# snuspl/rnb

Hardware: AMD Instinct MI355X
Metric: videos/sec (whole node) + p50/p99 end-to-end latency, R(2+1)D-34 8-frame clips (higher is better)
Workload: dtype fp32

## Files before the change

### csrc/conv_h3.hip

```cpp
#include <type_traits>
#include <hip/hip_runtime.h>
#include <stdint.h>

#include "x6d_common.h"

#include "h3_common.h"

#ifdef H3_PHASE_TIMING
__device__ unsigned long long* h3_phase_buf;
#define H3_PHASE(k)                                                                   \
  do {                                                                                \
    if (threadIdx.x == 0 && (k) < 16) {                                               \
      h3_phase_buf[(size_t)blockIdx.x * 16 + (k)] = __builtin_amdgcn_s_memtime();     \
      if ((k) == 0) {                                                                 \
        unsigned hw, xcc;                                                             \
        asm volatile("s_getreg_b32 %0, hwreg(HW_REG_HW_ID)" : "=s"(hw));              \
        asm volatile("s_getreg_b32 %0, hwreg(HW_REG_XCC_ID)" : "=s"(xcc));            \
        h3_phase_buf[(size_t)blockIdx.x * 16 + 14] = ((unsigned long long)xcc << 32) | hw; \
      }                                                                               \
    }                                                                                 \
  } while (0)
#else
#define H3_PHASE(k) do {} while (0)
#endif
// ... 764 lines not shown
      rd_w(wh[0], wl[0], half * G, 0);
#pragma unroll
      for (int j = 0; j < G; ++j) {
        if (t0 + j >= 9) break;
        const bool more = j + 1 < G && t0 + j + 1 < 9;
#pragma unroll
        for (int tc = 0; tc < TC; ++tc) {
          const int cs = (j * TC + tc) & 1;
          if (tc + 1 < TC) rd_w(wh[cs ^ 1], wl[cs ^ 1], half * G + j, tc + 1);
          else if (more) rd_w(wh[cs ^ 1], wl[cs ^ 1], half * G + j + 1, 0);
          if (more && tc >= 1 && tc <= TP) rd_bf(bf[(j + 1) & 1][tc - 1], t0 + j + 1, tc - 1);
          const H3B (&b)[TP] = bf[j & 1];
#pragma unroll
          for (int tp = 0; tp < TP; ++tp) acc[tp][tc] = h3_mma(wl[cs], b[tp].h, acc[tp][tc]);
#pragma unroll
          for (int tp = 0; tp < TP; ++tp) acc[tp][tc] = h3_mma(wh[cs], b[tp].l, acc[tp][tc]);
#pragma unroll
          for (int tp = 0; tp < TP; ++tp) acc[tp][tc] = h3_mma(wh[cs], b[tp].h, acc[tp][tc]);
          __builtin_amdgcn_sched_barrier(0);
        }
      }
      x6d_wait_vm<0>();
      x6d_barrier();
      half ^= 1;
    }
    H3_PHASE(2 + 2 * c);
  }
  x6d_epilogue<TP, TC, NW, C_TILE, ST, STK>(p, st, acc, p0, m_end, p0 + P_TILE, c0, wave, 0,
                                            lane, lds, HALO_BYTES + 2 * G * W_BYTES,
                                            st.out_scale);
  H3_PHASE(15);
}

template <int NW, int TP, int TC, int HALO, int WB, int MINB, bool ST, bool AFF>
__global__ __launch_bounds__(64 * NW, MINB)
void conv_h3t_kernel(const ConvF32Params p, const X6DStats st) {
  constexpr int ROWS = NW * TP * 16, C_TILE = TC * 16;
  constexpr int HALO_BYTES = HALO * 128;
  constexpr int TAP_BYTES = C_TILE * 128;
  constexpr int W_BYTES = 3 * TAP_BYTES;
  constexpr int W_TOTAL = W_BYTES / 1024;
  constexpr int W_INSTR = (W_TOTAL + NW - 1) / NW;
  constexpr int NT = 64 * NW;
  constexpr int ITEMS = (HALO * 4 + NT - 1) / NT;
  static_assert(NT % 4 == 0 && TAP_BYTES % 1024 == 0, "staging / DMA split");
  static_assert(TP <= TC * 3 - 1, "next-tap fragments are read during the channel tiles");
  __shared__ __attribute__((aligned(16))) char lds[HALO_BYTES + WB * W_BYTES];
  char* const wbuf = lds + HALO_BYTES;

  const int lane = threadIdx.x & 63;
  const int wave = __builtin_amdgcn_readfirstlane(threadIdx.x >> 6);
  const int frow = lane & 15, fq = lane >> 4;
  const int T = p.T, HW = p.H * p.W, P = p.ngroups;
  const int nck = (p.Cin_p + 31) / 32;

  const int nwg = gridDim.x, bid = blockIdx.x;
  const int q8 = nwg >> 3, r8 = nwg & 7, xcd = bid & 7;
  const int wgid = (xcd < r8 ? xcd * (q8 + 1) : r8 * (q8 + 1) + (xcd - r8) * q8) + (bid >> 3);
  const int ctile = wgid % p.n_ctiles;
  const int rest = wgid / p.n_ctiles;
  const int ptile = rest % p.n_ptiles;
  const int n = rest / p.n_ptiles;
  const int c0 = ctile * C_TILE, hw0 = ptile * P;

  const x6d_u32x4 wr = x6d_rsrc(p.w, (uint32_t)(p.K_pad / 32) * (uint32_t)p.w_rows * 128u);
  auto issue_w = [&](int c, int buf) {
#pragma unroll
    for (int j = 0; j < W_INSTR; ++j) {
      const int instr = (W_TOTAL % NW == 0) ? wave + NW * j : min(wave + NW * j, W_TOTAL - 1);
      const int k = instr / (TAP_BYTES / 1024), part = instr % (TAP_BYTES / 1024);
      const uint32_t s = (uint32_t)(k * nck + c);
      x6d_dma16(wr, (s * (uint32_t)p.w_rows + (uint32_t)c0) * 128u +
                        (uint32_t)(part * 1024 + lane * 16),
                wbuf + buf * W_BYTES + instr * 1024);
    }
  };

  const __amdgpu_buffer_rsrc_t xr =
      __builtin_amdgcn_make_buffer_rsrc((void*)p.x, (short)0, p.x_bytes, 0x00020000);
  const int nent = (T + 2) * P;
  const int qd = threadIdx.x & 3;
  uint32_t src[ITEMS];
  int dst[ITEMS];
#pragma unroll
  for (int i = 0; i < ITEMS; ++i) {
    const int it = threadIdx.x + i * NT;
    const int e = it >> 2;
    const int fr = e / P - 1, px = e - (fr + 1) * P;
    const bool ok = it < 4 * nent && fr >= 0 && fr < T && hw0 + px < HW;
    src[i] = ok ? (uint32_t)((((n * T + fr) * HW + hw0 + px) * p.Cin_p + qd * 4) * 4) : X6D_INVALID;
    dst[i] = it < 4 * nent ? e * 128 : -1;
  }
  const float* ssv = nullptr;
  if constexpr (AFF) ssv = st.in_ss + (size_t)st.in_seg[n] * 2 * p.Cin_p + qd * 4;
  const float in_scale = st.in_scale;
  x6f32x4 raw0[ITEMS], raw1[ITEMS];
  auto load_chunk = [&](int c) {
    const bool hi_ok = c * 32 + 16 < p.Cin_p;
#pragma unroll
    for (int i = 0; i < ITEMS; ++i) {
      const uint32_t o = src[i] == X6D_INVALID ? X6D_INVALID : src[i] + (uint32_t)(c * 128);
      raw0[i] = __builtin_amdgcn_raw_buffer_load_b128(xr, o, 0, 0);
      raw1[i] = __builtin_amdgcn_raw_buffer_load_b128(xr, (o == X6D_INVALID || !hi_ok) ? X6D_INVALID
                                                                                  : o + 64u, 0, 0);
    }
  };
  auto store_chunk = [&](int c) {
    x6f32x4 sc0, sh0, sc1, sh1;
    if constexpr (AFF) {
      const bool hi_ok = c * 32 + 16 < p.Cin_p;
      const float* ss = ssv + c * 32;
      sc0 = *(const x6f32x4*)ss;
      sh0 = *(const x6f32x4*)(ss + p.Cin_p);
      sc1 = hi_ok ? *(const x6f32x4*)(ss + 16) : (x6f32x4){0.f, 0.f, 0.f, 0.f};
      sh1 = hi_ok ? *(const x6f32x4*)(ss + p.Cin_p + 16) : (x6f32x4){0.f, 0.f, 0.f, 0.f};
    }
#pragma unroll
    for (int i = 0; i < ITEMS; ++i) {
      if (dst[i] < 0) continue;
      const int e = dst[i] >> 7;
      x6f32x4 a0 = raw0[i], a1 = raw1[i];
      if constexpr (AFF) {
        const float m = src[i] == X6D_INVALID ? 0.f : in_scale;
#pragma unroll
        for (int j = 0; j < 4; ++j) {
          a0[j] = fmaxf(fmaf(a0[j], sc0[j], sh0[j]), 0.f) * m;
          a1[j] = fmaxf(fmaf(a1[j], sc1[j], sh1[j]), 0.f) * m;
        }
      } else {
        a0 *= in_scale;
        a1 *= in_scale;
      }
      uint32_t h[4], l[4];
      h3_split4(a0, h, l);
      h3_split4(a1, h + 2, l + 2);
      char* base = lds + dst[i];
      *(wu32x4*)(base + (x6r_swz(2 * qd, e) << 4)) = (wu32x4){h[0], h[1], h[2], h[3]};
      *(wu32x4*)(base + (x6r_swz(2 * qd + 1, e) << 4)) = (wu32x4){l[0], l[1], l[2], l[3]};
    }
  };

  int pe[TP];
#pragma unroll
  for (int tp = 0; tp < TP; ++tp) {
    const int r = (wave * TP + tp) * 16 + frow;
    const int fr = r / P;
    pe[tp] = fr * P + (r - fr * P);
  }

  x6f32x4 acc[TP][TC];
#pragma unroll
  for (int b = 0; b < TC; ++b) {
    const int c = c0 + b * 16 + 4 * fq;
    const float4 b4 = *(const float4*)(p.bias + c);
    const x6f32x4 bv = (x6f32x4){b4.x, b4.y, b4.z, b4.w} * st.acc_scale;
#pragma unroll
    for (int a = 0; a < TP; ++a) acc[a][b] = bv;
  }
  const int w_hh = x6_chunk(2 * fq, frow) << 4, w_ll = x6_chunk(2 * fq + 1, frow) << 4;
  auto rd_bf = [&](H3B& b, int k, int tp) {
    const int e = pe[tp] + k * P;
    const char* base = lds + e * 128;
    b.h = *(const wu32x4*)(base + (x6r_swz(2 * fq, e) << 4));
    b.l = *(const wu32x4*)(base + (x6r_swz(2 * fq + 1, e) << 4));
  };
  auto rd_w = [&](wu32x4& ah, wu32x4& al, int buf, int k, int tc) {
    const char* wrow = wbuf + buf * W_BYTES + k * TAP_BYTES + (tc * 16 + frow) * 128;
    ah = *(const wu32x4*)(wrow + w_hh);
    al = *(const wu32x4*)(wrow + w_ll);
  };

  int buf = 0;
  auto taps = [&]() {
    H3B bf[2][TP];
    wu32x4 wh[2], wl[2];
#pragma unroll
    for (int tp = 0; tp < TP; ++tp) rd_bf(bf[0][tp], 0, tp);
    rd_w(wh[0], wl[0], buf, 0, 0);
#pragma unroll
    for (int k = 0; k < 3; ++k) {
#pragma unroll
      for (int tc = 0; tc < TC; ++tc) {
        const int cs = (k * TC + tc) & 1;
        if (tc + 1 < TC) rd_w(wh[cs ^ 1], wl[cs ^ 1], buf, k, tc + 1);
        else if (k + 1 < 3) rd_w(wh[cs ^ 1], wl[cs ^ 1], buf, k + 1, 0);
        if (k + 1 < 3) {
#pragma unroll
          for (int tp = 0; tp < TP; ++tp)
            if (tp * TC / TP == tc && tp < TP) rd_bf(bf[(k + 1) & 1][tp], k + 1, tp);
        }
        const H3B (&b)[TP] = bf[k & 1];
#pragma unroll
        for (int tp = 0; tp < TP; ++tp) acc[tp][tc] = h3_mma(wl[cs], b[tp].h, acc[tp][tc]);
#pragma unroll
        for (int tp = 0; tp < TP; ++tp) acc[tp][tc] = h3_mma(wh[cs], b[tp].l, acc[tp][tc]);
#pragma unroll
        for (int tp = 0; tp < TP; ++tp) acc[tp][tc] = h3_mma(wh[cs], b[tp].h, acc[tp][tc]);
        __builtin_amdgcn_sched_barrier(0);
      }
    }
  };
  issue_w(0, 0);
  load_chunk(0);
  for (int c = 0; c < nck; ++c) {
    if (c > 0) x6d_barrier();
    if (WB == 1 && c > 0) issue_w(c, 0);
    store_chunk(c);
    x6d_wait_vm<0>();
    x6d_barrier();
    if (c + 1 < nck) {
      if (WB == 2) issue_w(c + 1, (c + 1) & 1);
      load_chunk(c + 1);
    }
    buf = WB == 2 ? (c & 1) : 0;
    taps();
  }

  const float out_scale = st.out_scale;
  const uint32_t y_bytes = (uint32_t)p.M * (uint32_t)p.y_stride * 4u;
  const __amdgpu_buffer_rsrc_t yr =
      __builtin_amdgcn_make_buffer_rsrc((void*)p.y, (short)0, y_bytes, 0x00020000);
  const bool has_res = p.res != nullptr;
  const __amdgpu_buffer_rsrc_t rr = __builtin_amdgcn_make_buffer_rsrc(
      (void*)(has_res ? p.res : p.y), (short)0,
      has_res ? (uint32_t)p.M * (uint32_t)p.res_stride * 4u : 0u, 0x00020000);
  int mrow[TP];
#pragma unroll
  for (int tp = 0; tp < TP; ++tp) {
    const int r = (wave * TP + tp) * 16 + frow;
    const int fr = r / P, px = r - fr * P;
    mrow[tp] = hw0 + px < HW ? (n * T + fr) * HW + hw0 + px : -1;
  }
  double* red = (double*)lds;
  bool bad = false;
  if constexpr (ST) {
    x6d_barrier();
    for (int i = threadIdx.x; i < C_TILE * 2; i += NT) red[i] = 0.0;
    __syncthreads();
  }
#pragma unroll
  for (int tc = 0; tc < TC; ++tc) {
    const int cl = tc * 16 + 4 * fq, c = c0 + cl;
    x6f32x4 rv[TP];
#pragma unroll
    for (int tp = 0; tp < TP; ++tp) {
      const bool ok = has_res && mrow[tp] >= 0 && c < p.Cout_p;
      rv[tp] = has_res ? __builtin_amdgcn_raw_buffer_load_b128(
                             rr, ok ? (uint32_t)(mrow[tp] * p.res_stride + c) * 4u : X6D_INVALID,
                             0, 0)
                       : (x6f32x4){0.f, 0.f, 0.f, 0.f};
    }
    float s1[4] = {0.f, 0.f, 0.f, 0.f}, s2[4] = {0.f, 0.f, 0.f, 0.f};
#pragma unroll
    for (int tp = 0; tp < TP; ++tp) {
      const bool ok = mrow[tp] >= 0 && c < p.Cout_p;
      x6f32x4 v = acc[tp][tc] * out_scale + rv[tp];
      if (st.oflag != nullptr && ok) bad |= x6d_nonfinite(v);
      if (p.relu) {
#pragma unroll
        for (int j = 0; j < 4; ++j) v[j] = fmaxf(v[j], 0.f);
      }
      __builtin_amdgcn_raw_buffer_store_b128(
          v, yr, ok ? (uint32_t)(mrow[tp] * p.y_stride + c) * 4u : X6D_INVALID, 0, 0);
      if (ST && ok) {
#pragma unroll
        for (int j = 0; j < 4; ++j) {
          s1[j] += v[j];
// ... 330 lines not shown
  f32_magic_div((uint32_t)p.Ho, &p.mHo, &p.sHo);
  f32_magic_div((uint32_t)p.To, &p.mTo, &p.sTo);
  f32_magic_div((uint32_t)p.H + 1u, &p.mG, &p.sG);
  p.ST = R;
  p.n_ctiles = (p.Cout_p + 143) / 144;
  if (p.n_ctiles * 144 > p.w_rows) return -8;
  const long long blocks = rnb_conv_h3r_blocks(variant, p.N, p.T, p.H, p.W, p.Cout_p);
  if (blocks > 0x7FFFFFFF) return -7;
  if (sums && (!clip_seg || stats_c < p.Cout_p)) return -12;
  X6DStats st;
  st.sums = sums;
  st.clip_seg = clip_seg;
  st.stats_c = stats_c;
  st.ksplit = 1;
  st.ws = nullptr;
  st.in_scale = in_scale;
  st.out_scale = out_scale;
  st.acc_scale = 1.f / out_scale;
  st.in_ss = in_ss;
  st.in_seg = in_seg;
  st.oflag = g_h3_range_flag;
  const int kid = (sums ? 1 : 0) + (in_ss ? 2 : 0);
  hipLaunchKernelGGL(stacked ? cfg.stacked[kid] : cfg.kernel[kid], dim3((unsigned)blocks),
                     dim3(64 * cfg.nw), 0, stream, p, st);
  return (int)hipGetLastError();
}

struct ConvH3TConfig {
  int rows, c_tile, halo, nw;
  void (*kernel)(const ConvF32Params, const X6DStats);
  void (*kernel_st)(const ConvF32Params, const X6DStats);
  void (*kernel_aff)(const ConvF32Params, const X6DStats);
  void (*kernel_aff_st)(const ConvF32Params, const X6DStats);
};
#define H3TCFG(NW, TP, TC, HALO, WB, MINB)                                         \
  {NW * TP * 16, TC * 16, HALO, NW,                                                  \
   conv_h3t_kernel<NW, TP, TC, HALO, WB, MINB, false, false>,                       \
   conv_h3t_kernel<NW, TP, TC, HALO, WB, MINB, true, false>,                        \
   conv_h3t_kernel<NW, TP, TC, HALO, WB, MINB, false, true>,                        \
   conv_h3t_kernel<NW, TP, TC, HALO, WB, MINB, true, true>}
static const ConvH3TConfig kH3TConfigs[] = {
    H3TCFG(8, 4, 4, 768, 2, 1), H3TCFG(8, 2, 4, 512, 2, 1), H3TCFG(8, 2, 8, 512, 2, 1),
    H3TCFG(4, 4, 4, 384, 1, 2),
};

int rnb_conv_h3t_num_variants() { return (int)(sizeof(kH3TConfigs) / sizeof(kH3TConfigs[0])); }

int rnb_conv_h3t_pixels(int variant, int T) {
  if (variant < 0 || variant >= rnb_conv_h3t_num_variants() || T < 2) return 0;
  const ConvH3TConfig& cfg = kH3TConfigs[variant];
  if (cfg.rows % T) return 0;
  const int P = cfg.rows / T;
  return (P % 16 == 0 && (T + 2) * P <= cfg.halo) ? P : 0;
}

int rnb_conv_h3t_launch(const ConvF32Params* pp, int variant, hipStream_t stream, double* sums,
                        const int* clip_seg, int stats_c, float in_scale, float out_scale,
                        const float* in_ss, const int* in_seg) {
  if (variant < 0 || variant >= rnb_conv_h3t_num_variants()) return -1;
  ConvF32Params p = *pp;
  const ConvH3TConfig& cfg = kH3TConfigs[variant];
  if (p.KT != 3 || p.KH != 1 || p.KW != 1 || p.PT != 1 || p.PH != 0 || p.PW != 0) return -2;
  if (p.ST != 1 || p.SH != 1 || p.SW != 1 || p.Cin_p % 16 != 0 || p.Cout_p % 4 != 0) return -2;
  const int nck = (p.Cin_p + 31) / 32;
  if (p.K_pad != 3 * 32 * nck) return -3;
  if (p.M <= 0) return 0;
  if (p.M != p.N * p.T * p.H * p.W) return -3;
  if (p.y_stride < p.Cout_p || p.y_stride % 4 != 0 || (p.res && (p.res_stride < p.Cout_p ||
                                                               p.res_stride % 4 != 0)))
    return -4;
  const long long xb = (long long)p.N * p.T * p.H * p.W * p.Cin_p * 4;
  if (xb > 0x7FFFFF00LL || (long long)p.M * p.y_stride * 4 > 0x7FFFFF00LL) return -5;
  if (p.res && (long long)p.M * p.res_stride * 4 > 0x7FFFFF00LL) return -6;
  const int P = rnb_conv_h3t_pixels(variant, p.T);
  if (P == 0) return -13;
  if ((long long)(p.K_pad / 32) * p.w_rows * 128 > 0x7FFFFF00LL) return -11;
  if (!(in_scale > 0.f) || !(out_scale > 0.f)) return -15;
  if (in_ss && !in_seg) return -16;
  p.x_bytes = (uint32_t)xb;
  p.ngroups = P;
  p.n_ptiles = (p.H * p.W + P - 1) / P;
  p.n_ctiles = (p.Cout_p + cfg.c_tile - 1) / cfg.c_tile;
  if (p.n_ctiles * cfg.c_tile > p.w_rows) return -8;
  const long long blocks = (long long)p.N * p.n_ptiles * p.n_ctiles;
  if (blocks > 0x7FFFFFFF) return -7;
  if (sums && (!clip_seg || stats_c < p.Cout_p)) return -12;
  X6DStats st;
  st.sums = sums;
  st.clip_seg = clip_seg;
  st.stats_c = stats_c;
  st.ksplit = 1;
  st.ws = nullptr;
  st.in_scale = in_scale;
  st.out_scale = out_scale;
  st.acc_scale = 1.f / out_scale;
  st.in_ss = in_ss;
  st.in_seg = in_seg;
  st.oflag = g_h3_range_flag;
  const bool aff = in_ss != nullptr;
  hipLaunchKernelGGL(aff ? (sums ? cfg.kernel_aff_st : cfg.kernel_aff)
                         : (sums ? cfg.kernel_st : cfg.kernel),
                     dim3((unsigned)blocks), dim3(64 * cfg.nw), 0, stream, p, st);
  return (int)hipGetLastError();
}

}
```

### rnb_amd/ops/conv_f32.py

```python
from __future__ import annotations

import math
import os
from typing import Dict, Optional, Tuple

import torch
import torch.nn.functional as F

from . import tuning
from .conv import ConvGeom, pad_to

F32_ALIGN = 4
F32_BK = 32
F32_ROW_SLACK = 256


_DEV_NAMES: Dict[int, str] = {}


def _device_name(device) -> str:
    if device is None or getattr(device, "type", "cpu") != "cuda":
        return "cpu"
    idx = device.index if device.index is not None else torch.cuda.current_device()
    if idx not in _DEV_NAMES:
# ... 390 lines not shown
            b[:self.geom.cout] = self.bias[:self.geom.cout].cpu()
            sw = h3_weight_scale_log2(w)
            self._h3d = (h3_direct_weights(w, sw).to(self.device), b.to(self.device),
                         float(2.0 ** H3_IN_LOG2), float(2.0 ** -(H3_IN_LOG2 + sw)))
        return self._h3d

    @property
    def h3t_k_pad(self) -> int:
        return 3 * 32 * ((self.geom.cin_p + 31) // 32)

    def h3t_buffers(self):
        if self.geom.cin_p % 32 == 0:
            return self.h3d_buffers()
        if self._h3t is None:
            rows, cin, kp = self.geom.cout_p + X6_ROW_SLACK, self.geom.cin_p, self.h3t_k_pad
            w = torch.zeros(rows, kp, dtype=torch.float32)
            tap = kp // 3
            src = self.wmat[:self.geom.cout, :self.k_total].cpu()
            for k in range(3):
                w[:self.geom.cout, k * tap:k * tap + cin] = src[:, k * cin:(k + 1) * cin]
            b = torch.zeros(rows, dtype=torch.float32)
            b[:self.geom.cout] = self.bias[:self.geom.cout].cpu()
            sw = h3_weight_scale_log2(w)
            self._h3t = (h3_direct_weights(w, sw).to(self.device), b.to(self.device),
                         float(2.0 ** H3_IN_LOG2), float(2.0 ** -(H3_IN_LOG2 + sw)))
        return self._h3t

    def h3t_ok(self, x_shape=None) -> bool:
        return (self.winot_ok and self.geom.cin_p % 16 == 0
                and (x_shape is None or x_shape[1] >= 2))

    def h3t_fits(self, variant: int, x_shape) -> bool:
        from .native import kernels
        return x_shape is None or kernels().conv_h3t_pixels(variant, x_shape[1]) > 0

    def h3p_ok(self, x_shape=None) -> bool:
        if not self.h3t_ok(x_shape) or os.environ.get("RNB_H3P", "1") == "0":
            return False
        from .native import kernels
        if x_shape is None:
            return kernels().conv_h3p_ok(8, 16, 16, self.geom.cin_p, self.geom.cout_p)
        _, T, H, W, _ = x_shape
        return kernels().conv_h3p_ok(T, H, W, self.geom.cin_p, self.geom.cout_p)

    def h3u_fits(self, variant: int, x_shape) -> bool:
        from .native import kernels
        return x_shape is None or kernels().conv_h3u_pixels(variant, x_shape[1]) > 0

    def wino_u(self, tc: int, m: int = 2, co0: int = 0, nco: Optional[int] = None,
               x6: bool = False) -> torch.Tensor:
        nco = self.geom.cout_p - co0 if nco is None else nco
        key = (m, tc, co0, nco, x6)
        u = self._wino_u.get(key)
        if u is None:
            fn = {2: winograd_weights, -4: winograd_t_weights}[m]
            w = self.w_ref[co0:co0 + nco].cpu()
            if w.shape[1] < self.geom.cin_p:
                w = torch.cat([w, w.new_zeros((w.shape[0], self.geom.cin_p - w.shape[1])
                                              + tuple(w.shape[2:]))], dim=1)
            u = self._wino_u[key] = fn(w, nco, tc, x6=x6).to(self.device)
        return u

    def h3w_u(self, tc: int) -> Tuple[torch.Tensor, int]:
        got = self._h3w.get(tc)
        if got is None:
            u, sw = h3w_weights(self.w_ref, self.geom.cin_p, self.geom.cout_p, tc)
            got = self._h3w[tc] = (u.to(self.device), sw)
# ... 643 lines not shown
```

### rnb_amd/ops/native.py

```python
from __future__ import annotations

import ctypes
import os
import struct
import threading
from typing import Optional

_HERE = os.path.dirname(os.path.abspath(__file__))
NATIVE_DIR = os.path.join(os.path.dirname(_HERE), "_native")

_lock = threading.Lock()
_libs = {}


class NativeUnavailable(RuntimeError):
    pass


def _lib_path(name: str) -> str:
    return os.path.join(NATIVE_DIR, name)


def _load(name: str, build_if_missing: bool = True) -> ctypes.CDLL:
    with _lock:
# ... 324 lines not shown
                                            ctypes.c_void_p, ctypes.c_void_p,
                                            ctypes.c_void_p, ctypes.c_int]
        lib.rnb_conv_x6r_launch.restype = ctypes.c_int
        lib.rnb_conv_x6_config_info.argtypes = [ctypes.c_int, ctypes.POINTER(ctypes.c_int),
                                                ctypes.POINTER(ctypes.c_int)]
        lib.rnb_conv_h3_launch.argtypes = [ctypes.POINTER(ConvParams), ctypes.c_int,
                                           ctypes.c_void_p, ctypes.c_void_p, ctypes.c_void_p,
                                           ctypes.c_int, ctypes.c_int, ctypes.c_void_p,
                                           ctypes.c_float, ctypes.c_float, ctypes.c_void_p,
                                           ctypes.c_void_p]
        lib.rnb_conv_h3_launch.restype = ctypes.c_int
        lib.rnb_conv_h3_affine_ok.argtypes = [ctypes.c_int, ctypes.c_int, ctypes.c_int]
        lib.rnb_conv_h3_affine_ok.restype = ctypes.c_int
        lib.rnb_conv_h3r_launch.argtypes = [ctypes.POINTER(ConvParams), ctypes.c_int,
                                            ctypes.c_void_p, ctypes.c_void_p, ctypes.c_void_p,
                                            ctypes.c_int, ctypes.c_float, ctypes.c_float,
                                            ctypes.c_void_p, ctypes.c_void_p]
        lib.rnb_conv_h3r_launch.restype = ctypes.c_int
        lib.rnb_conv_h3r_band_rows.argtypes = [ctypes.c_int] * 3
        lib.rnb_conv_h3r_band_rows.restype = ctypes.c_int
        lib.rnb_conv_h3r_pixels.argtypes = [ctypes.c_int]
        lib.rnb_conv_h3r_pixels.restype = ctypes.c_int
        lib.rnb_conv_h3r_blocks.argtypes = [ctypes.c_int] * 6
        lib.rnb_conv_h3r_blocks.restype = ctypes.c_longlong
        lib.rnb_conv_h3r_stacked.argtypes = [ctypes.c_int] * 6
        lib.rnb_conv_h3r_stacked.restype = ctypes.c_int
        lib.rnb_conv_h3r_stack_small.argtypes = [ctypes.c_int]
        lib.rnb_conv_h3r_stack_small.restype = None
        lib.rnb_conv_h3r_occupancy.argtypes = [ctypes.c_int] * 2
        lib.rnb_conv_h3r_occupancy.restype = ctypes.c_int
        lib.rnb_conv_h3t_launch.argtypes = lib.rnb_conv_h3r_launch.argtypes
        lib.rnb_conv_h3t_launch.restype = ctypes.c_int
        lib.rnb_conv_h3t_pixels.argtypes = [ctypes.c_int, ctypes.c_int]
        self.exp = None
        exp_path = os.path.join(NATIVE_DIR, "exp", "librnb_h3exp.so")
        if os.path.exists(exp_path) and os.environ.get("RNB_EXP_KERNELS", "1") != "0":
            try:
                self.exp = ctypes.CDLL(exp_path)
            except OSError:
                self.exp = None
        if self.exp is not None:
            ex = self.exp
            ex.rnb_conv_h3u_launch.argtypes = lib.rnb_conv_h3r_launch.argtypes
            ex.rnb_conv_h3u_launch.restype = ctypes.c_int
            ex.rnb_conv_h3u_pixels.argtypes = [ctypes.c_int, ctypes.c_int]
            ex.rnb_conv_h3u_pixels.restype = ctypes.c_int
            ex.rnb_conv_h3s_launch.argtypes = [ctypes.POINTER(ConvParams), ctypes.c_int,
                                               ctypes.c_void_p, ctypes.c_void_p,
                                               ctypes.c_void_p, ctypes.c_int, ctypes.c_float,
                                               ctypes.c_float]
            ex.rnb_conv_h3s_launch.restype = ctypes.c_int
            ex.rnb_conv_h3s_rows.argtypes = [ctypes.c_int, ctypes.c_int, ctypes.c_int]
            ex.rnb_conv_h3s_rows.restype = ctypes.c_int
        lib.rnb_conv_h3stem_launch.argtypes = [ctypes.POINTER(ConvParams), ctypes.c_int,
                                               ctypes.c_void_p, ctypes.c_void_p,
                                               ctypes.c_void_p, ctypes.c_int, ctypes.c_float,
                                               ctypes.c_float]
        lib.rnb_conv_h3stem_launch.restype = ctypes.c_int
        lib.rnb_conv_h3stem_rows.argtypes = [ctypes.c_int, ctypes.c_int, ctypes.c_int]
        lib.rnb_conv_h3stem_rows.restype = ctypes.c_int
        lib.rnb_conv_h3p_launch.argtypes = [ctypes.POINTER(ConvParams), ctypes.c_int,
                                            ctypes.c_void_p, ctypes.c_void_p, ctypes.c_void_p,
                                            ctypes.c_int, ctypes.c_float, ctypes.c_float,
                                            ctypes.c_void_p, ctypes.c_void_p]
        lib.rnb_conv_h3p_launch.restype = ctypes.c_int
        lib.rnb_conv_h3p_ok.argtypes = [ctypes.c_int] * 5
# ... 158 lines not shown

    def conv_h3p(self, params: ConvParams, blocks_per_cu: int, stream: int, in_scale: float,
                 out_scale: float, sums: int = 0, clip_seg: int = 0, stats_c: int = 0,
                 in_ss: int = 0, in_seg: int = 0) -> None:
        _check(self.lib.rnb_conv_h3p_launch(ctypes.byref(params), blocks_per_cu, stream,
                                            sums or None, clip_seg or None, stats_c, in_scale,
                                            out_scale, in_ss or None, in_seg or None),
               "conv_h3p (%d blocks per CU)" % blocks_per_cu)

    def conv_h3w(self, params: "WinoParams", variant: int, stream: int, in_scale: float,
                 out_scale: float, out_seg: int = 0) -> None:
        _check(self.lib.rnb_conv_h3w_launch(ctypes.byref(params), variant, stream, in_scale,
                                            out_scale, out_seg or None),
               "conv_h3w (variant %d)" % variant)

    def conv_h3w_tc(self, variant: int) -> int:
        return int(self.lib.rnb_conv_h3w_tc(variant))

    def conv_h3p_ok(self, T: int, H: int, W: int, Cin_p: int, Cout_p: int) -> bool:
        return bool(self.lib.rnb_conv_h3p_ok(T, H, W, Cin_p, Cout_p))

    def conv_h3stem_rows(self, variant: int, Ho: int, Wo: int) -> int:
        return int(self.lib.rnb_conv_h3stem_rows(variant, Ho, Wo))

    def conv_h3s_rows(self, variant: int, Ho: int, Wo: int) -> int:
        return int(self.exp.rnb_conv_h3s_rows(variant, Ho, Wo)) if self.exp else 0

    def conv_h3u_pixels(self, variant: int, T: int) -> int:
        return int(self.exp.rnb_conv_h3u_pixels(variant, T)) if self.exp else 0

    def conv_h3t_pixels(self, variant: int, T: int) -> int:
        return int(self.lib.rnb_conv_h3t_pixels(variant, T))

    def conv_h3_affine_ok(self, config_id: int, cin_p: int, rows_per_clip: int) -> bool:
        return bool(self.lib.rnb_conv_h3_affine_ok(config_id, cin_p, rows_per_clip))

    def conv_x6r(self, params: ConvParams, variant: int, stream: int, sums: int = 0,
                 clip_seg: int = 0, stats_c: int = 0) -> None:
        _check(self.lib.rnb_conv_x6r_launch(ctypes.byref(params), variant, stream,
                                            sums or None, clip_seg or None, stats_c),
               "conv_x6r (variant %d)" % variant)

    def wino_f32(self, params: "WinoParams", variant: int, stream: int) -> None:
        _check(self.lib.rnb_wino_f32_launch(ctypes.byref(params), variant, stream),
               "conv_wino_f32 (variant %d)" % variant)

    def winot_f32(self, params: "WinoParams", variant: int, stream: int) -> None:
        _check(self.lib.rnb_winot_f32_launch(ctypes.byref(params), variant, stream),
               "conv_winot_f32 (variant %d)" % variant)

    def wino_x6(self, params: "WinoParams", variant: int, stream: int) -> None:
        _check(self.lib.rnb_wino_x6_launch(ctypes.byref(params), variant, stream),
               "conv_wino_x6 (variant %d)" % variant)

    def winot_x6(self, params: "WinoParams", variant: int, stream: int) -> None:
        _check(self.lib.rnb_winot_x6_launch(ctypes.byref(params), variant, stream),
               "conv_winot_x6 (variant %d)" % variant)

    def preprocess_f32(self, in_ptr, out_ptr, npix, mean, std, stream):
        m = (ctypes.c_float * 3)(*mean)
        s = (ctypes.c_float * 3)(*std)
        _check(self.lib.rnb_preprocess_f32(in_ptr, out_ptr, npix, m, s, stream),
               "preprocess_f32")

    def head_f32(self, x_ptr, w_ptr, b_ptr, out_ptr, pooled_ptr, N, S, C, Cs, ncls, stream):
        _check(self.lib.rnb_head_f32(x_ptr, w_ptr, b_ptr, out_ptr, pooled_ptr, N, S, C, Cs,
# ... 538 lines not shown
```

Measured before the change: 1653.

## Add stacked-clip tiling to temporal h3t conv, skipping padded temporal taps

Adds a stacked form of the temporal (3x1x1) conv kernel. A block's rows now span pixels from several clips across all frames, with no per-clip padding, so layers with small H*W or short T fill whole tiles. The padding frames are dropped from the halo, and a tap-skipping inner loop leaves out MMAs that would only read zero temporal padding. Frame order is reversed per wave to line up the skipped taps. A new epilogue handles stores and per-segment BN statistics when one block holds several clips. The host picks the stacked form when it needs fewer blocks. The cost is more complex indexing, extra template instantiations, and a slower statistics fallback when a block mixes many segments.

Result: faster. 1675, median of 6 (+1.3%).

```diff
diff --git a/csrc/conv_h3.hip b/csrc/conv_h3.hip
--- a/csrc/conv_h3.hip
+++ b/csrc/conv_h3.hip
@@ -820,10 +820,11 @@
   H3_PHASE(15);
 }
 
-template <int NW, int TP, int TC, int HALO, int WB, int MINB, bool ST, bool AFF>
+template <int NW, int TP, int TC, int HALO, int WB, int MINB, bool ST, bool AFF, int STK = 0>
 __global__ __launch_bounds__(64 * NW, MINB)
 void conv_h3t_kernel(const ConvF32Params p, const X6DStats st) {
   constexpr int ROWS = NW * TP * 16, C_TILE = TC * 16;
+  static_assert(!STK || HALO == ROWS, "stacked: the patch is the block's T x P rows");
   constexpr int HALO_BYTES = HALO * 128;
   constexpr int TAP_BYTES = C_TILE * 128;
   constexpr int W_BYTES = 3 * TAP_BYTES;
@@ -870,6 +871,27 @@
   const int qd = threadIdx.x & 3;
   uint32_t src[ITEMS];
   int dst[ITEMS];
+  [[maybe_unused]] const int NG = p.N * HW, lgP = 31 - __clz(P);
+  [[maybe_unused]] int n0 = 0, n1 = 0;
+  [[maybe_unused]] bool mixed = false;
+  if constexpr (STK) {
+    n0 = __builtin_amdgcn_readfirstlane(f32_fast_div(hw0, p.mG, p.sG));
+    n1 = __builtin_amdgcn_readfirstlane(f32_fast_div(min(hw0 + P, NG) - 1, p.mG, p.sG));
+    if constexpr (AFF) mixed = st.in_seg[n0] != st.in_seg[n1];
+#pragma unroll
+    for (int i = 0; i < ITEMS; ++i) {
+      const int e = (threadIdx.x + i * NT) >> 2;
+      const int fr = e >> lgP, g = hw0 + (e & (P - 1));
+      const int nn = f32_fast_div(g, p.mG, p.sG);
+      const bool ok = g < NG;
+      src[i] = ok ? (uint32_t)((((nn * T + fr) * HW + (g - nn * HW)) * p.Cin_p + qd * 4) * 4)
+                  : X6D_INVALID;
+      dst[i] = e * 128;
+      if constexpr (AFF) {
+        if (ok) dst[i] |= (nn - n0) << 17;
+      }
+    }
+  } else {
 #pragma unroll
   for (int i = 0; i < ITEMS; ++i) {
     const int it = threadIdx.x + i * NT;
@@ -879,8 +901,9 @@
     src[i] = ok ? (uint32_t)((((n * T + fr) * HW + hw0 + px) * p.Cin_p + qd * 4) * 4) : X6D_INVALID;
     dst[i] = it < 4 * nent ? e * 128 : -1;
   }
+  }
   const float* ssv = nullptr;
-  if constexpr (AFF) ssv = st.in_ss + (size_t)st.in_seg[n] * 2 * p.Cin_p + qd * 4;
+  if constexpr (AFF) ssv = st.in_ss + (size_t)st.in_seg[STK ? n0 : n] * 2 * p.Cin_p + qd * 4;
   const float in_scale = st.in_scale;
   x6f32x4 raw0[ITEMS], raw1[ITEMS];
   auto load_chunk = [&](int c) {
@@ -906,8 +929,19 @@
 #pragma unroll
     for (int i = 0; i < ITEMS; ++i) {
       if (dst[i] < 0) continue;
-      const int e = dst[i] >> 7;
+      const int e = (STK && AFF ? dst[i] & 0x1FFFF : dst[i]) >> 7;
       x6f32x4 a0 = raw0[i], a1 = raw1[i];
+      if constexpr (STK && AFF) {
+        if (mixed) {
+          const bool hi_ok = c * 32 + 16 < p.Cin_p;
+          const float* ss = st.in_ss + qd * 4 + c * 32 +
+                            (size_t)st.in_seg[n0 + (dst[i] >> 17)] * 2 * p.Cin_p;
+          sc0 = *(const x6f32x4*)ss;
+          sh0 = *(const x6f32x4*)(ss + p.Cin_p);
+          sc1 = hi_ok ? *(const x6f32x4*)(ss + 16) : (x6f32x4){0.f, 0.f, 0.f, 0.f};
+          sh1 = hi_ok ? *(const x6f32x4*)(ss + p.Cin_p + 16) : (x6f32x4){0.f, 0.f, 0.f, 0.f};
+        }
+      }
       if constexpr (AFF) {
         const float m = src[i] == X6D_INVALID ? 0.f : in_scale;
 #pragma unroll
@@ -922,19 +956,37 @@
       uint32_t h[4], l[4];
       h3_split4(a0, h, l);
       h3_split4(a1, h + 2, l + 2);
-      char* base = lds + dst[i];
+      char* base = lds + (STK && AFF ? dst[i] & 0x1FFFF : dst[i]);
       *(wu32x4*)(base + (x6r_swz(2 * qd, e) << 4)) = (wu32x4){h[0], h[1], h[2], h[3]};
       *(wu32x4*)(base + (x6r_swz(2 * qd + 1, e) << 4)) = (wu32x4){l[0], l[1], l[2], l[3]};
     }
   };
 
   int pe[TP];
+  [[maybe_unused]] int tf[TP], tq[TP], sg = 1;
+  if constexpr (STK) {
+    int fb = 0;
+    if constexpr (STK == 1) {
+      fb = (wave * TP * 16) >> lgP;
+      sg = fb ? -1 : 1;
+    } else if constexpr (STK == 3) {
+      sg = (wave & 1) ? -1 : 1;
+      fb = (wave & 1) ? T - 1 : 0;
+    }
+#pragma unroll
+    for (int tp = 0; tp < TP; ++tp) {
+      tf[tp] = STK == 1 ? fb : fb + sg * tp;
+      tq[tp] = STK == 1 ? ((wave * TP + tp) * 16) & (P - 1) : (STK == 3 ? wave >> 1 : wave) * 16;
+      pe[tp] = (tf[tp] - sg) * P + tq[tp] + frow;
+    }
+  } else {
 #pragma unroll
   for (int tp = 0; tp < TP; ++tp) {
     const int r = (wave * TP + tp) * 16 + frow;
     const int fr = r / P;
     pe[tp] = fr * P + (r - fr * P);
   }
+  }
 
   x6f32x4 acc[TP][TC];
 #pragma unroll
@@ -947,13 +999,14 @@
   }
   const int w_hh = x6_chunk(2 * fq, frow) << 4, w_ll = x6_chunk(2 * fq + 1, frow) << 4;
   auto rd_bf = [&](H3B& b, int k, int tp) {
-    const int e = pe[tp] + k * P;
+    const int e = pe[tp] + k * (STK ? sg * P : P);
     const char* base = lds + e * 128;
     b.h = *(const wu32x4*)(base + (x6r_swz(2 * fq, e) << 4));
     b.l = *(const wu32x4*)(base + (x6r_swz(2 * fq + 1, e) << 4));
   };
   auto rd_w = [&](wu32x4& ah, wu32x4& al, int buf, int k, int tc) {
-    const char* wrow = wbuf + buf * W_BYTES + k * TAP_BYTES + (tc * 16 + frow) * 128;
+    const char* wrow = wbuf + buf * W_BYTES + (STK ? 1 + sg * (k - 1) : k) * TAP_BYTES +
+                       (tc * 16 + frow) * 128;
     ah = *(const wu32x4*)(wrow + w_hh);
     al = *(const wu32x4*)(wrow + w_ll);
   };
@@ -984,6 +1037,45 @@
         for (int tp = 0; tp < TP; ++tp) acc[tp][tc] = h3_mma(wh[cs], b[tp].l, acc[tp][tc]);
 #pragma unroll
         for (int tp = 0; tp < TP; ++tp) acc[tp][tc] = h3_mma(wh[cs], b[tp].h, acc[tp][tc]);
+        __builtin_amdgcn_sched_barrier(0);
+      }
+    }
+  };
+  [[maybe_unused]] auto taps_skip = [&]() {
+    constexpr int ALL = (1 << TP) - 1;
+    constexpr int M0 = STK == 1 ? ALL : 1, M2 = STK == 2 ? 1 << (TP - 1) : 0;
+    constexpr int K0 = M0 == ALL ? 1 : 0, K1 = M2 == ALL ? 2 : 3;
+    auto on = [](int k, int tp) constexpr {
+      return !((k == 0 ? M0 : k == 2 ? M2 : 0) >> tp & 1);
+    };
+    H3B bf[2][TP];
+    wu32x4 wh[2], wl[2];
+#pragma unroll
+    for (int tp = 0; tp < TP; ++tp)
+      if (on(K0, tp)) rd_bf(bf[K0 & 1][tp], K0, tp);
+    rd_w(wh[0], wl[0], buf, K0, 0);
+#pragma unroll
+    for (int k = K0; k < K1; ++k) {
+#pragma unroll
+      for (int tc = 0; tc < TC; ++tc) {
+        const int cs = ((k - K0) * TC + tc) & 1;
+        if (tc + 1 < TC) rd_w(wh[cs ^ 1], wl[cs ^ 1], buf, k, tc + 1);
+        else if (k + 1 < K1) rd_w(wh[cs ^ 1], wl[cs ^ 1], buf, k + 1, 0);
+        if (k + 1 < K1) {
+#pragma unroll
+          for (int tp = 0; tp < TP; ++tp)
+            if (tp * TC / TP == tc && on(k + 1, tp)) rd_bf(bf[(k + 1) & 1][tp], k + 1, tp);
+        }
+        const H3B (&b)[TP] = bf[k & 1];
+#pragma unroll
+        for (int tp = 0; tp < TP; ++tp)
+          if (on(k, tp)) acc[tp][tc] = h3_mma(wl[cs], b[tp].h, acc[tp][tc]);
+#pragma unroll
+        for (int tp = 0; tp < TP; ++tp)
+          if (on(k, tp)) acc[tp][tc] = h3_mma(wh[cs], b[tp].l, acc[tp][tc]);
+#pragma unroll
+        for (int tp = 0; tp < TP; ++tp)
+          if (on(k, tp)) acc[tp][tc] = h3_mma(wh[cs], b[tp].h, acc[tp][tc]);
         __builtin_amdgcn_sched_barrier(0);
       }
     }
@@ -1001,7 +1093,8 @@
       load_chunk(c + 1);
     }
     buf = WB == 2 ? (c & 1) : 0;
-    taps();
+    if constexpr (STK) taps_skip();
+    else taps();
   }
 
   const float out_scale = st.out_scale;
@@ -1013,14 +1106,147 @@
       (void*)(has_res ? p.res : p.y), (short)0,
       has_res ? (uint32_t)p.M * (uint32_t)p.res_stride * 4u : 0u, 0x00020000);
   int mrow[TP];
+  double* red = (double*)lds;
+  bool bad = false;
+  if constexpr (STK) {
+    constexpr int LDS_BYTES = HALO_BYTES + WB * W_BYTES, CQ = C_TILE / 4;
+    [[maybe_unused]] int sl[TP];
+    int seg_lo = 0, nseg = 1;
+    if constexpr (ST) {
+      seg_lo = __builtin_amdgcn_readfirstlane(st.clip_seg[n0]);
+      nseg = __builtin_amdgcn_readfirstlane(st.clip_seg[n1]) - seg_lo + 1;
+    }
+    const bool in_lds = nseg * C_TILE * 16 <= LDS_BYTES;
+    const bool uni = nseg <= X6D_MSEG_MAX && in_lds;
+#pragma unroll
+    for (int tp = 0; tp < TP; ++tp) {
+      const int g = hw0 + tq[tp] + frow;
+      const int nn = f32_fast_div(g, p.mG, p.sG);
+      mrow[tp] = g < NG ? (nn * T + tf[tp]) * HW + (g - nn * HW) : -1;
+      if constexpr (ST) {
+        sl[tp] = g < NG ? 0 : -1;
+        if (nseg > 1 && uni && g < NG) sl[tp] = st.clip_seg[nn] - seg_lo;
+      }
+    }
+    if constexpr (ST) {
+      x6d_barrier();
+      if (in_lds)
+        for (int i = threadIdx.x; i < nseg * C_TILE * 2; i += NT) red[i] = 0.0;
+      __syncthreads();
+    }
+#pragma unroll
+    for (int tc = 0; tc < TC; ++tc) {
+      const int cl = tc * 16 + 4 * fq, c = c0 + cl;
+      x6f32x4 rv[TP];
+#pragma unroll
+      for (int tp = 0; tp < TP; ++tp) {
+        const bool ok = has_res && mrow[tp] >= 0 && c < p.Cout_p;
+        rv[tp] = has_res ? __builtin_amdgcn_raw_buffer_load_b128(
+                               rr, ok ? (uint32_t)(mrow[tp] * p.res_stride + c) * 4u : X6D_INVALID,
+                               0, 0)
+                         : (x6f32x4){0.f, 0.f, 0.f, 0.f};
+      }
+      float s1[4] = {0.f, 0.f, 0.f, 0.f}, s2[4] = {0.f, 0.f, 0.f, 0.f};
+#pragma unroll
+      for (int tp = 0; tp < TP; ++tp) {
+        const bool ok = mrow[tp] >= 0 && c < p.Cout_p;
+        x6f32x4 v = acc[tp][tc] * out_scale + rv[tp];
+        if (st.oflag != nullptr && ok) bad |= x6d_nonfinite(v);
+        if (p.relu) {
+#pragma unroll
+          for (int j = 0; j < 4; ++j) v[j] = fmaxf(v[j], 0.f);
+        }
+        __builtin_amdgcn_raw_buffer_store_b128(
+            v, yr, ok ? (uint32_t)(mrow[tp] * p.y_stride + c) * 4u : X6D_INVALID, 0, 0);
+        rv[tp] = v;
+        if (ST && ok) {
+#pragma unroll
+          for (int j = 0; j < 4; ++j) {
+            s1[j] += v[j];
+            s2[j] = fmaf(v[j], v[j], s2[j]);
+          }
+        }
+      }
+      if constexpr (ST) {
+        if (uni) {
+#pragma unroll 1
+          for (int s = 0; s < nseg; ++s) {
+            if (nseg > 1) {
+#pragma unroll
+              for (int j = 0; j < 4; ++j) s1[j] = s2[j] = 0.f;
+#pragma unroll
+              for (int tp = 0; tp < TP; ++tp) {
+                if (sl[tp] != s) continue;
+#pragma unroll
+                for (int j = 0; j < 4; ++j) {
+                  s1[j] += rv[tp][j];
+                  s2[j] = fmaf(rv[tp][j], rv[tp][j], s2[j]);
+                }
+              }
+            }
+#pragma unroll
+            for (int j = 0; j < 4; ++j) {
+              s1[j] = x6d_row16_sum(s1[j]);
+              s2[j] = x6d_row16_sum(s2[j]);
+            }
+            if (frow == 0 && c < p.Cout_p) {
+#pragma unroll
+              for (int j = 0; j < 4; ++j) {
+                atomicAdd(red + (s * C_TILE + cl + j) * 2, (double)s1[j]);
+                atomicAdd(red + (s * C_TILE + cl + j) * 2 + 1, (double)s2[j]);
+              }
+            }
+          }
+        }
+      }
+    }
+    if constexpr (ST) {
+      if (!uni) {
+        asm volatile("s_waitcnt vmcnt(0)" ::: "memory");
+        __syncthreads();
+#pragma unroll 1
+        for (int i = threadIdx.x; i < ROWS * CQ; i += NT) {
+          const int e = i / CQ, cl = (i % CQ) * 4, c = c0 + cl;
+          const int g = hw0 + (e & (P - 1));
+          if (g >= NG || c >= p.Cout_p) continue;
+          const int nn = f32_fast_div(g, p.mG, p.sG);
+          const int m = (nn * T + (e >> lgP)) * HW + (g - nn * HW);
+          const x6f32x4 v = __builtin_amdgcn_raw_buffer_load_b128(
+              yr, (uint32_t)(m * p.y_stride + c) * 4u, 0, 1);
+          const int sg = st.clip_seg[nn];
+#pragma unroll 1
+          for (int j = 0; j < 4; ++j) {
+            const double a = (double)v[j], b = (double)v[j] * (double)v[j];
+            if (in_lds) {
+              atomicAdd(red + ((size_t)(sg - seg_lo) * C_TILE + cl + j) * 2, a);
+              atomicAdd(red + ((size_t)(sg - seg_lo) * C_TILE + cl + j) * 2 + 1, b);
+            } else {
+              atomicAdd(st.sums + ((size_t)sg * 2) * st.stats_c + c + j, a);
+              atomicAdd(st.sums + ((size_t)sg * 2 + 1) * st.stats_c + c + j, b);
+            }
+          }
+        }
+      }
+      __syncthreads();
+      if (in_lds) {
+        for (int i = threadIdx.x; i < nseg * C_TILE; i += NT) {
+          const int sg = seg_lo + i / C_TILE, c = c0 + i % C_TILE;
+          if (c < p.Cout_p) {
+            atomicAdd(st.sums + ((size_t)sg * 2) * st.stats_c + c, red[i * 2]);
+            atomicAdd(st.sums + ((size_t)sg * 2 + 1) * st.stats_c + c, red[i * 2 + 1]);
+          }
+        }
+      }
+    }
+    if (bad) *st.oflag = 1;
+    return;
+  }
 #pragma unroll
   for (int tp = 0; tp < TP; ++tp) {
     const int r = (wave * TP + tp) * 16 + frow;
     const int fr = r / P, px = r - fr * P;
     mrow[tp] = hw0 + px < HW ? (n * T + fr) * HW + hw0 + px : -1;
   }
-  double* red = (double*)lds;
-  bool bad = false;
   if constexpr (ST) {
     x6d_barrier();
     for (int i = threadIdx.x; i < C_TILE * 2; i += NT) red[i] = 0.0;
@@ -1417,15 +1643,30 @@
   void (*kernel_st)(const ConvF32Params, const X6DStats);
   void (*kernel_aff)(const ConvF32Params, const X6DStats);
   void (*kernel_aff_st)(const ConvF32Params, const X6DStats);
+  int tp;
+  void (*stacked[3][4])(const ConvF32Params, const X6DStats);
 };
-#define H3TCFG(NW, TP, TC, HALO, WB, MINB)                                         \
-  {NW * TP * 16, TC * 16, HALO, NW,                                                  \
+#define H3TSTK(NW, TP, TC, WB, MINB, STK)                                           \
+  {conv_h3t_kernel<NW, TP, TC, NW * TP * 16, WB, MINB, false, false, STK>,          \
+   conv_h3t_kernel<NW, TP, TC, NW * TP * 16, WB, MINB, true, false, STK>,           \
+   conv_h3t_kernel<NW, TP, TC, NW * TP * 16, WB, MINB, false, true, STK>,           \
+   conv_h3t_kernel<NW, TP, TC, NW * TP * 16, WB, MINB, true, true, STK>}
+#define H3TPC(NW, TP, TC, HALO, WB, MINB)                                           \
+  NW * TP * 16, TC * 16, HALO, NW,                                                   \
    conv_h3t_kernel<NW, TP, TC, HALO, WB, MINB, false, false>,                       \
    conv_h3t_kernel<NW, TP, TC, HALO, WB, MINB, true, false>,                        \
    conv_h3t_kernel<NW, TP, TC, HALO, WB, MINB, false, true>,                        \
-   conv_h3t_kernel<NW, TP, TC, HALO, WB, MINB, true, true>}
+   conv_h3t_kernel<NW, TP, TC, HALO, WB, MINB, true, true>, TP
+#define H3TCFG(NW, TP, TC, HALO, WB, MINB)                                          \
+  {H3TPC(NW, TP, TC, HALO, WB, MINB),                                               \
+   {H3TSTK(NW, TP, TC, WB, MINB, 1), H3TSTK(NW, TP, TC, WB, MINB, 2),               \
+    H3TSTK(NW, TP, TC, WB, MINB, 3)}}
+#define H3TCFG_TP2(NW, TC, HALO, WB, MINB)                                          \
+  {H3TPC(NW, 2, TC, HALO, WB, MINB),                                                \
+   {H3TSTK(NW, 2, TC, WB, MINB, 1), {nullptr, nullptr, nullptr, nullptr},           \
+    H3TSTK(NW, 2, TC, WB, MINB, 3)}}
 static const ConvH3TConfig kH3TConfigs[] = {
-    H3TCFG(8, 4, 4, 768, 2, 1), H3TCFG(8, 2, 4, 512, 2, 1), H3TCFG(8, 2, 8, 512, 2, 1),
+    H3TCFG(8, 4, 4, 768, 2, 1), H3TCFG_TP2(8, 4, 512, 2, 1), H3TCFG_TP2(8, 8, 512, 2, 1),
     H3TCFG(4, 4, 4, 384, 1, 2),
 };
 
@@ -1437,6 +1678,55 @@
   if (cfg.rows % T) return 0;
   const int P = cfg.rows / T;
   return (P % 16 == 0 && (T + 2) * P <= cfg.halo) ? P : 0;
+}
+
+static int g_h3t_form = 0;
+void rnb_conv_h3t_form(int mode) { g_h3t_form = mode; }
+
+static long long h3t_blocks(int variant, long long N, int T, int H, int W, int Cout_p,
+                            int* stacked) {
+  *stacked = 0;
+  if (variant < 0 || variant >= rnb_conv_h3t_num_variants()) return 0;
+  if (N < 1 || T < 2 || H < 1 || W < 1 || Cout_p < 1) return 0;
+  const ConvH3TConfig& cfg = kH3TConfigs[variant];
+  if (cfg.rows % T) return 0;
+  const int P = cfg.rows / T;
+  if (P % 16) return 0;
+  const long long HW = (long long)H * W;
+  const bool fits_pc = (T + 2) * P <= cfg.halo;
+  const int stk_form = T == 2 ? 1 : T == cfg.tp ? 2 : T == 2 * cfg.tp ? 3 : 0;
+  const bool fits_stk = stk_form && (P & (P - 1)) == 0 && N * HW + P <= 0x7FFFFFFFLL;
+  if (!fits_pc && !fits_stk) return 0;
+  const long long n_ctiles = (Cout_p + cfg.c_tile - 1) / cfg.c_tile;
+  const long long pc = N * ((HW + P - 1) / P) * n_ctiles;
+  const long long stk = (N * HW + P - 1) / P * n_ctiles;
+  bool on;
+  if (!fits_pc) on = true;
+  else if (!fits_stk) on = false;
+  else if (g_h3t_form != 0) on = g_h3t_form > 0;
+  else on = stk < pc;
+  *stacked = on ? stk_form : 0;
+  return on ? stk : pc;
+}
+
+int rnb_conv_h3t_stacked(int variant, int N, int T, int H, int W, int Cout_p) {
+  int stacked;
+  h3t_blocks(variant, N, T, H, W, Cout_p, &stacked);
+  return stacked ? 1 : 0;
+}
+
+long long rnb_conv_h3t_blocks(int variant, int N, int T, int H, int W, int Cout_p) {
+  int stacked;
+  return h3t_blocks(variant, N, T, H, W, Cout_p, &stacked);
+}
+
+int rnb_conv_h3t_occupancy(int variant, int stacked) {
+  if (variant < 0 || variant >= rnb_conv_h3t_num_variants()) return -1;
+  const ConvH3TConfig& cfg = kH3TConfigs[variant];
+  int nb = 0;
+  const hipError_t e = hipOccupancyMaxActiveBlocksPerMultiprocessor(
+      &nb, (const void*)(stacked ? cfg.stacked[0][0] : cfg.kernel), 64 * cfg.nw, 0);
+  return e == hipSuccess ? nb : -(int)e;
 }
 
 int rnb_conv_h3t_launch(const ConvF32Params* pp, int variant, hipStream_t stream, double* sums,
@@ -1457,17 +1747,19 @@
   const long long xb = (long long)p.N * p.T * p.H * p.W * p.Cin_p * 4;
   if (xb > 0x7FFFFF00LL || (long long)p.M * p.y_stride * 4 > 0x7FFFFF00LL) return -5;
   if (p.res && (long long)p.M * p.res_stride * 4 > 0x7FFFFF00LL) return -6;
-  const int P = rnb_conv_h3t_pixels(variant, p.T);
-  if (P == 0) return -13;
+  int stacked;
+  const long long blocks = h3t_blocks(variant, p.N, p.T, p.H, p.W, p.Cout_p, &stacked);
+  if (blocks == 0) return -13;
+  const int P = cfg.rows / p.T;
   if ((long long)(p.K_pad / 32) * p.w_rows * 128 > 0x7FFFFF00LL) return -11;
   if (!(in_scale > 0.f) || !(out_scale > 0.f)) return -15;
   if (in_ss && !in_seg) return -16;
   p.x_bytes = (uint32_t)xb;
   p.ngroups = P;
-  p.n_ptiles = (p.H * p.W + P - 1) / P;
   p.n_ctiles = (p.Cout_p + cfg.c_tile - 1) / cfg.c_tile;
+  p.n_ptiles = stacked ? (int)(blocks / p.n_ctiles) : (p.H * p.W + P - 1) / P;
+  f32_magic_div((uint32_t)(p.H * p.W), &p.mG, &p.sG);
   if (p.n_ctiles * cfg.c_tile > p.w_rows) return -8;
-  const long long blocks = (long long)p.N * p.n_ptiles * p.n_ctiles;
   if (blocks > 0x7FFFFFFF) return -7;
   if (sums && (!clip_seg || stats_c < p.Cout_p)) return -12;
   X6DStats st;
@@ -1483,8 +1775,9 @@
   st.in_seg = in_seg;
   st.oflag = g_h3_range_flag;
   const bool aff = in_ss != nullptr;
-  hipLaunchKernelGGL(aff ? (sums ? cfg.kernel_aff_st : cfg.kernel_aff)
-                         : (sums ? cfg.kernel_st : cfg.kernel),
+  hipLaunchKernelGGL(stacked ? cfg.stacked[stacked - 1][(sums ? 1 : 0) + (aff ? 2 : 0)]
+                     : aff   ? (sums ? cfg.kernel_aff_st : cfg.kernel_aff)
+                             : (sums ? cfg.kernel_st : cfg.kernel),
                      dim3((unsigned)blocks), dim3(64 * cfg.nw), 0, stream, p, st);
   return (int)hipGetLastError();
 }
diff --git a/rnb_amd/ops/conv_f32.py b/rnb_amd/ops/conv_f32.py
--- a/rnb_amd/ops/conv_f32.py
+++ b/rnb_amd/ops/conv_f32.py
@@ -446,7 +446,10 @@
 
     def h3t_fits(self, variant: int, x_shape) -> bool:
         from .native import kernels
-        return x_shape is None or kernels().conv_h3t_pixels(variant, x_shape[1]) > 0
+        if x_shape is None:
+            return True
+        N, T, H, W, _ = x_shape
+        return kernels().conv_h3t_blocks(variant, N, T, H, W, self.geom.cout_p) > 0
 
     def h3p_ok(self, x_shape=None) -> bool:
         if not self.h3t_ok(x_shape) or os.environ.get("RNB_H3P", "1") == "0":
diff --git a/rnb_amd/ops/native.py b/rnb_amd/ops/native.py
--- a/rnb_amd/ops/native.py
+++ b/rnb_amd/ops/native.py
@@ -380,6 +380,14 @@
         lib.rnb_conv_h3t_launch.argtypes = lib.rnb_conv_h3r_launch.argtypes
         lib.rnb_conv_h3t_launch.restype = ctypes.c_int
         lib.rnb_conv_h3t_pixels.argtypes = [ctypes.c_int, ctypes.c_int]
+        lib.rnb_conv_h3t_blocks.argtypes = [ctypes.c_int] * 6
+        lib.rnb_conv_h3t_blocks.restype = ctypes.c_longlong
+        lib.rnb_conv_h3t_stacked.argtypes = [ctypes.c_int] * 6
+        lib.rnb_conv_h3t_stacked.restype = ctypes.c_int
+        lib.rnb_conv_h3t_form.argtypes = [ctypes.c_int]
+        lib.rnb_conv_h3t_form.restype = None
+        lib.rnb_conv_h3t_occupancy.argtypes = [ctypes.c_int] * 2
+        lib.rnb_conv_h3t_occupancy.restype = ctypes.c_int
         self.exp = None
         exp_path = os.path.join(NATIVE_DIR, "exp", "librnb_h3exp.so")
         if os.path.exists(exp_path) and os.environ.get("RNB_EXP_KERNELS", "1") != "0":
@@ -604,6 +612,19 @@
     def conv_h3t_pixels(self, variant: int, T: int) -> int:
         return int(self.lib.rnb_conv_h3t_pixels(variant, T))
 
+    def conv_h3t_blocks(self, variant: int, N: int, T: int, H: int, W: int, cout_p: int) -> int:
+        return int(self.lib.rnb_conv_h3t_blocks(variant, N, T, H, W, cout_p))
+
+    def conv_h3t_stacked(self, variant: int, N: int, T: int, H: int, W: int,
+                         cout_p: int) -> bool:
+        return bool(self.lib.rnb_conv_h3t_stacked(variant, N, T, H, W, cout_p))
+
+    def conv_h3t_form(self, mode: int) -> None:
+        self.lib.rnb_conv_h3t_form(mode)
+
+    def conv_h3t_occupancy(self, variant: int, stacked: bool) -> int:
+        return self.lib.rnb_conv_h3t_occupancy(variant, 1 if stacked else 0)
+
     def conv_h3_affine_ok(self, config_id: int, cin_p: int, rows_per_clip: int) -> bool:
         return bool(self.lib.rnb_conv_h3_affine_ok(config_id, cin_p, rows_per_clip))
 
```
